# quanpn90/avsr

Measured on AMD Instinct MI355X. Metric: AV-frames/sec/GPU (fwd+bwd) on 15s clips; WER parity on LRS2 test, higher is better.
Workload: dtype bf16

## Files before the change

### avsr_amd/_lib.py

```python
import ctypes
import os

import torch

_HERE = os.path.dirname(os.path.abspath(__file__))
LIB_PATH = os.environ.get("AVSR_LIB_PATH_AB") or os.path.join(_HERE, "libavsr_hip.so")

AVSR_F32, AVSR_BF16 = 0, 1
ACT_NONE, ACT_GELU, ACT_RELU = 0, 1, 2

_c_p = ctypes.c_void_p
_i64 = ctypes.c_int64
_f = ctypes.c_float
_i = ctypes.c_int


class GemmParams(ctypes.Structure):
    _fields_ = [
        ("M", _i), ("N", _i), ("K", _i), ("batch", _i),
        ("dtype", _i), ("a_kmajor", _i), ("b_kmajor", _i), ("c_f32", _i),
        ("A", _c_p), ("lda", _i64), ("strideA", _i64),
        ("B", _c_p), ("ldb", _i64), ("strideB", _i64),
        ("C", _c_p), ("ldc", _i64), ("strideC", _i64),
        ("alpha", _f), ("beta", _f),
# ... 175 lines not shown


class BeamSelectParams(ctypes.Structure):
    _fields_ = [
        ("n", _i), ("V", _i), ("P", _i), ("beam", _i), ("blank", _i), ("eos", _i), ("w_dec", _f), ("w_ctc", _f),
        ("dec", _c_p), ("ld", _i64), ("ids", _c_p), ("psi", _c_p), ("s_prev", _c_p), ("score", _c_p),
        ("out_prev", _c_p), ("out_tok", _c_p), ("out_col", _c_p), ("out_score", _c_p), ("out_dec", _c_p),
        ("out_ctc", _c_p), ("out_s", _c_p), ("nseg", _i), ("seg", _c_p),
    ]


class BeamPostParams(ctypes.Structure):
    _fields_ = [
        ("U", _i), ("beam", _i), ("P", _i), ("R", _i), ("Lmax", _i), ("steps_cap", _i), ("eos", _i),
        ("end_detect", _i), ("d_end", ctypes.c_double), ("pos", _c_p), ("maxlen", _c_p),
        ("sel_prev", _c_p), ("sel_tok", _c_p), ("sel_col", _c_p), ("sel_score", _c_p), ("sel_dec", _c_p),
        ("sel_ctc", _c_p), ("sel_s", _c_p),
        ("tok", _c_p), ("score", _c_p), ("sdec", _c_p), ("sctc", _c_p), ("s_prev", _c_p), ("src", _c_p),
        ("bp_prev", _c_p), ("bp_tok", _c_p), ("end_flag", _c_p), ("end_score", _c_p), ("end_dec", _c_p),
        ("end_ctc", _c_p), ("best_len", _c_p), ("best_end", _c_p), ("done", _c_p),
    ]


class FbankParams(ctypes.Structure):
    _fields_ = [
        ("B", _i), ("T", _i), ("wav", _c_p), ("ldw", _i64), ("n_samples", _c_p),
        ("bins", _i * 28), ("preemph", _f), ("ln_eps", _f), ("out", _c_p),
    ]


class TimeMaskParams(ctypes.Structure):
    _fields_ = [("B", _i), ("L", _i), ("nspan", _i), ("row_bytes", _i64), ("clip_stride_bytes", _i64),
                ("x", _c_p), ("spans", _c_p)]


class AddNoiseParams(ctypes.Structure):
    _fields_ = [("B", _i), ("L", _i), ("x", _c_p), ("ldx", _i64), ("noise", _c_p), ("ldn", _i64),
                ("lengths", _c_p), ("snr_db", _c_p), ("y", _c_p), ("ldy", _i64), ("ws", _c_p)]


class VideoNormParams(ctypes.Structure):
    _fields_ = [
        ("B", _i), ("T", _i), ("H", _i), ("W", _i), ("crop", _i), ("oy", _i), ("ox", _i),
        ("frames", _c_p), ("mean", _f), ("std", _f), ("out", _c_p),
    ]


SYMBOLS = {
    "avsr_version": ([], ctypes.c_char_p),
    "avsr_set_option": ([_i, _i64], _i),
    "avsr_get_option": ([_i], _i64),
    "avsr_gemm": ([ctypes.POINTER(GemmParams), _c_p], _i),
    "avsr_gemm_wgrad_group": ([ctypes.POINTER(GemmParams), _i, _c_p], _i),
    "avsr_gemm_skinny_splits": ([_i, _i, _i], _i),
    "avsr_conv_fwd": ([ctypes.POINTER(ConvParams), _c_p], _i),
    "avsr_conv_bwd_data": ([ctypes.POINTER(ConvParams), _c_p], _i),
    "avsr_conv_bwd_weight": ([ctypes.POINTER(ConvParams), _c_p], _i),
    "avsr_conv_stat_tiles": ([ctypes.POINTER(ConvParams)], _i),
    "avsr_conv_bnr_tiles": ([ctypes.POINTER(ConvParams)], _i),
    "avsr_conv_wgrad_ws": ([ctypes.POINTER(ConvParams)], _i64),
    "avsr_layernorm_fwd": ([ctypes.POINTER(LayerNormParams), _c_p], _i),
    "avsr_layernorm_bwd": ([ctypes.POINTER(LayerNormParams), _c_p], _i),
    "avsr_bn_finalize": ([ctypes.POINTER(BnFinalizeParams), _c_p], _i),
    "avsr_bn_act_fwd": ([ctypes.POINTER(BnActParams), _c_p], _i),
    "avsr_bn_act_bwd_reduce": ([ctypes.POINTER(BnActParams), _c_p], _i),
    "avsr_bn_bwd_apply": ([ctypes.POINTER(BnActParams), _c_p], _i),
    "avsr_stem_pool_fwd": ([ctypes.POINTER(StemPoolParams), _c_p], _i),
    "avsr_stem_pool_bwd_apply": ([ctypes.POINTER(StemPoolParams), _c_p], _i),
    "avsr_bn_bwd_finalize": ([ctypes.POINTER(BnActParams), _i, _c_p], _i),
    "avsr_avgpool_fwd": ([_i, _i, _i, _i, _c_p, _c_p, _c_p], _i),
    "avsr_avgpool_bwd": ([_i, _i, _i, _i, _c_p, _c_p, _c_p], _i),
    "avsr_attn_fwd": ([ctypes.POINTER(AttnParams), _c_p], _i),
    "avsr_debug_attn_stamps": ([_c_p], _i),
    "avsr_attn_bwd_prep": ([ctypes.POINTER(AttnParams), _c_p], _i),
    "avsr_attn_bwd": ([ctypes.POINTER(AttnParams), _c_p], _i),
    "avsr_attn_dropmask": ([ctypes.POINTER(AttnParams), _c_p], _i),
    "avsr_attn_path": ([ctypes.POINTER(AttnParams), _i], _i),
    "avsr_row_lse": ([ctypes.POINTER(XentParams), _c_p], _i),
    "avsr_lsm_fwd": ([ctypes.POINTER(XentParams), _c_p], _i),
    "avsr_lsm_bwd": ([ctypes.POINTER(XentParams), _c_p], _i),
    "avsr_ctc_fwd": ([ctypes.POINTER(CtcParams), _c_p], _i),
    "avsr_ctc_bwd": ([ctypes.POINTER(CtcParams), _c_p], _i),
    "avsr_ctc_align": ([ctypes.POINTER(CtcAlignParams), _c_p], _i),
    "avsr_loss_finalize": ([_i, _c_p, _i, _c_p, _c_p, _f, _i, _c_p, _c_p], _i),
    "avsr_ew_bwd": ([ctypes.POINTER(EwParams), _c_p], _i),
    "avsr_colsum_defer": ([_i], _i),
    "avsr_colsum_flush": ([_c_p], _i),
    "avsr_colsum_inline": ([_i], _i),
    "avsr_dropout_fwd": ([ctypes.POINTER(EwParams), _c_p], _i),
    "avsr_mask_rows": ([_i, _i, _i, _i, _c_p, _i64, _c_p, _c_p], _i),
    "avsr_embed_fwd": ([ctypes.POINTER(EmbedParams), _c_p], _i),
    "avsr_embed_bwd": ([ctypes.POINTER(EmbedParams), _c_p], _i),
    "avsr_cast": ([_i, _i, _i, _i, _c_p, _i64, _c_p, _i64, _f, _f, _c_p], _i),
    "avsr_cast_flat": ([_i, _i, _i64, _c_p, _c_p, _c_p], _i),
    "avsr_stem_pack": ([_i, _i, _i, _c_p, _c_p, _c_p], _i),
    "avsr_stem_wpack": ([_i, _c_p, _c_p, _c_p], _i),
    "avsr_stem_conv_tiles": ([_i, _i], _i),
    "avsr_stem_wpack2": ([_c_p, _c_p, _c_p], _i),
    "avsr_stem_conv_fwd": ([_i, _i, _c_p, _c_p, _c_p, _c_p, _c_p], _i),
    "avsr_stem_wgrad_unpack": ([_c_p, _c_p, _c_p], _i),
    "avsr_audio_pack": ([_i, _i, _i, _i, _c_p, _c_p, _c_p], _i),
    "avsr_weightnorm_fwd": ([_i, _i, _i, _i, _c_p, _c_p, _c_p, _c_p, _c_p], _i),
    "avsr_weightnorm_bwd": ([_i, _i, _i, _c_p, _c_p, _c_p, _c_p, _c_p, _c_p, _c_p, _c_p], _i),
    "avsr_sumsq": ([_c_p, _i64, _c_p, _c_p, _c_p], _i),
    "avsr_adamw": ([ctypes.POINTER(AdamWParams), _c_p], _i),
    "avsr_log_softmax_rows": ([_i, _i, _i, _c_p, _i64, _c_p, _i64, _c_p], _i),
    "avsr_dec_attn": ([ctypes.POINTER(DecAttnParams), _c_p], _i),
    "avsr_row_topk": ([ctypes.POINTER(TopkParams), _c_p], _i),
    "avsr_log_softmax_topk": ([_i, _i, _i, _c_p, _i64, _c_p, _i64, _i, _c_p, _c_p], _i),
    "avsr_ctc_prefix": ([ctypes.POINTER(CtcPrefixParams), _c_p], _i),
    "avsr_beam_select": ([ctypes.POINTER(BeamSelectParams), _c_p], _i),
    "avsr_beam_step_prep": ([_i, _i, _c_p, _c_p, _c_p, _c_p], _i),
    "avsr_beam_kv_put": ([_i, _i, _i, _c_p, _i64, _c_p, _c_p, _c_p, _c_p], _i),
    "avsr_beam_post": ([ctypes.POINTER(BeamPostParams), _c_p], _i),
    "avsr_gather_rows": ([_i, _i, _i64, _c_p, _i64, _i64, _c_p, _i64, _i64, _c_p, _c_p], _i),
    "avsr_fbank_stack": ([ctypes.POINTER(FbankParams), _c_p], _i),
    "avsr_video_normalize": ([ctypes.POINTER(VideoNormParams), _c_p], _i),
    "avsr_time_mask": ([ctypes.POINTER(TimeMaskParams), _c_p], _i),
    "avsr_add_noise": ([ctypes.POINTER(AddNoiseParams), _c_p], _i),
    "avsr_rgb_to_gray": ([_c_p, _c_p, _i64, _c_p], _i),
}

_lib = None


class AvsrLibError(RuntimeError):
    pass


def load():
    global _lib
    if _lib is not None:
        return _lib
    if not os.path.exists(LIB_PATH):
        raise AvsrLibError(f"{LIB_PATH} not built: run `python -c 'import __graft_entry__ as g; g.build()'`")
    lib = ctypes.CDLL(LIB_PATH, mode=ctypes.RTLD_GLOBAL)
    for name, (argtypes, restype) in SYMBOLS.items():
        if os.environ.get("AVSR_LIB_PATH_AB") and not hasattr(lib, name):
            continue
        fn = getattr(lib, name)
        fn.argtypes = argtypes
        fn.restype = restype
    _lib = lib
    return lib


def check(rc, op):
    if rc != 0:
        raise AvsrLibError(f"{op} failed with code {rc}")


OPTIONS = {"gemm_tile": 0, "attn_sq_fwd": 1, "attn_sq_bwd": 2, "wgrad_dual": 3, "conv_192": 4, "conv_s2phase": 5,
           "conv_patch": 6, "conv_wpatch": 7, "stem_pool_2x2": 8,
           "stem_wpatch": 9}
TILES = ["128", "256", "256x128", "128x256", "128s3", "128w8s3", "pp", "192", "192x256", "192w8s3", "64", "64s4"]
ATTN_PATHS = ["f32", "tiled", "resident", "sq", "enc"]


def set_option(name, value):
    if name == "gemm_tile" and not isinstance(value, int):
        value = 0 if value in (None, "auto") else TILES.index(value) + 1
    lib = load()
    prev = get_option(name)
    check(lib.avsr_set_option(OPTIONS[name], int(value)), f"avsr_set_option({name}, {value})")
    return prev


def get_option(name):
    return int(load().avsr_get_option(OPTIONS[name]))


_raw_stream = getattr(torch._C, "_cuda_getCurrentRawStream", None)
_get_device = getattr(torch._C, "_cuda_getDevice", None) or torch.cuda.current_device


def stream_ptr(device=None):
    if _raw_stream is not None:
        idx = _get_device() if device is None else torch.device(device).index
        if idx is None:
            idx = _get_device()
        return ctypes.c_void_p(_raw_stream(idx))
    return ctypes.c_void_p(torch.cuda.current_stream(device).cuda_stream)
```

### avsr_amd/csrc/attention_enc.hip

```cpp
#include "attention.h"

namespace attn {
namespace sq {
constexpr int KT = 64;
constexpr int NS = 3;
constexpr int IMGB = KT * 128;
constexpr int STAGEB = 2 * IMGB;
static_assert(4 * 32 * 65 * 4 <= NS * STAGEB, "store slabs exceed the ring");

typedef __attribute__((address_space(3))) void lds_void_t;

AVSR_DEV int swz(int row) { const int g = (row >> 1) & 7; return g ^ ((g & 1) << 2); }
AVSR_DEV __amdgpu_buffer_rsrc_t rsrc(const void* base, uint32_t bytes) {
  const uint64_t b = (uint64_t)(uintptr_t)base;
  const uint64_t ub = ((uint64_t)(uint32_t)__builtin_amdgcn_readfirstlane((uint32_t)(b >> 32)) << 32) |
                      (uint32_t)__builtin_amdgcn_readfirstlane((uint32_t)b);
  return __builtin_amdgcn_make_buffer_rsrc((void*)(uintptr_t)ub, (short)0, (int)__builtin_amdgcn_readfirstlane(bytes),
                                           0x00020000);
}
AVSR_DEV void dma16(__amdgpu_buffer_rsrc_t r, uint32_t voff, char* lds_wave_base) {
  const uint32_t m = __builtin_amdgcn_readfirstlane((uint32_t)(uintptr_t)(lds_void_t*)lds_wave_base);
  asm volatile("s_mov_b32 m0, %0\n\ts_nop 0\n\tbuffer_load_dwordx4 %1, %2, 0 offen lds" ::"s"(m), "v"(voff), "s"(r)
               : "memory", "m0");
}
// ... 309 lines not shown
  if (g_stamps != nullptr) {
    __syncthreads();
    stamp_part(3, 0);
  }
}

template <int DM>
__global__ __launch_bounds__(NTH) void attn_bwd_dkdv_kernel(AttnArgs a) {
  extern __shared__ __attribute__((aligned(16))) char smem[];
  char* Qs = smem;
  char* dOs = smem + IMG384;
  float* lss = (float*)(smem + 2 * IMG384);
  float* dls = lss + MAXR;
  char* Kw = smem + 2 * IMG384 + 2 * MAXR * 4;
  stamp_part(0, 1);
  const int bh = xcd_id(blockIdx.x, gridDim.x), b = bh / a.H, h = bh % a.H;
  const int tid = threadIdx.x, l = tid & 63, c = l & 31, hh = l >> 5;
  const int w = __builtin_amdgcn_readfirstlane(tid >> 6);
  Kw += w * 4096;
  const int kb0 = w * 32, key = kb0 + c;
  const bf16* Qg = (const bf16*)a.q + (int64_t)b * a.Lq * a.ldq + h * DH;
  const bf16* dOg = (const bf16*)a.dout + (int64_t)b * a.Lq * a.lddo + h * DH;
  const bf16* Kg = (const bf16*)a.k + ((int64_t)b * a.Lk + kb0) * a.ldk + h * DH;
  const bf16* V = (const bf16*)a.v + (int64_t)b * a.Lk * a.ldv + h * DH;
  if (kb0 < a.Lk) {
#pragma unroll
    for (int i = 0; i < 4; ++i) dma_piece(Kg, a.ldk, min(32, a.Lk - kb0), Kw, i, l);
  }
  dma_piece(Qg, a.ldq, a.Lq, Qs, w, l);
  dma_piece(dOg, a.lddo, a.Lq, dOs, w, l);
  {
    const float* f = (w < 6 ? a.lse : a.delta) + (int64_t)bh * a.Lq;
    dma4(rsrc(f, (uint32_t)(a.Lq * 4)), (uint32_t)((64 * (w % 6) + l) * 4), (char*)((w < 6 ? lss : dls) + 64 * (w % 6)));
  }
  bf16x8 vf[4];
#pragma unroll
  for (int s = 0; s < 4; ++s) vf[s] = ldrow_sel(V, a.ldv, key, a.Lk, s * 16 + 8 * hh);
#pragma unroll
  for (int s = 0; s < 4; ++s) asm volatile("" ::"v"(vf[s]));
#pragma unroll
  for (int r = 1; r < 4; ++r) {
    dma_piece(Qg, a.ldq, a.Lq, Qs, 12 * r + w, l);
    dma_piece(dOg, a.lddo, a.Lq, dOs, 12 * r + w, l);
  }
  round_barrier();
  if (tid < MAXR) lss[tid] *= LOG2E;
  const int klen = a.klen ? min(a.klen[b], a.Lk) : a.Lk;
  const bool active = kb0 < klen, kok = key < klen;
  const float sl2 = a.scale * LOG2E;
  const AttnDrop drop(a.drop_p, a.seed, a.B, a.H, a.Lq, a.Lk);
  const float dscale = DM ? drop.scale : 1.f;
  const uint32_t nG = DM == 1 ? drop.npair * GOLD : 0u;
  const uint32_t keyG = DM == 1 ? ((uint32_t)bh * (uint32_t)a.Lq * drop.npair + (uint32_t)(min(key, a.Lk - 1) >> 1)) * GOLD : 0u;
  const bool odd = c & 1;
  const uint64_t* mp = DM == 2 ? a.mq + ((int64_t)bh * a.mnqb * a.mnkb + w) * 16 + ((c & 3) + 4 * (c >> 3)) : nullptr;
  const int mstride = a.mnkb * 16;
  const bool mhi = (c >> 2) & 1;
  const int nt = (a.Lq + 31) >> 5;
  FragOff fo;
  fo.init(l);
  f32x16 dv0, dv1, dk0, dk1;
  zacc(dv0); zacc(dv1); zacc(dk0); zacc(dk1);
#pragma unroll
  for (int r = 0; r < 4; ++r) {
    if (r == 1) vmwait<4>();
    if (r == 2) vmwait<2>();
    if (r == 3) vmwait<0>();
    round_barrier();
    if (r == 0) stamp_part(1, 1);
    if (active) {
#pragma unroll
      for (int u = 0; u < 3; ++u) {
        const int t = 3 * r + u;
        if (t >= nt) break;
        const int qt0 = t * 32;
        uint32_t mbits = 0;
        if (DM == 2) {
          const uint64_t m64 = mp[(int64_t)t * mstride];
          mbits = (mhi ? (uint32_t)(m64 >> 32) : (uint32_t)m64) >> (4 * hh);
        }
        const char* Qt = Qs + t * 4096;
        const char* dOt = dOs + t * 4096;
        f32x16 sc, dp;
        zacc(sc); zacc(dp);
        uint32_t kz = 0;
        asm volatile("" : "+v"(kz));
        const char* Kt = Kw + kz;
#pragma unroll
        for (int s = 0; s < 4; ++s) {
          sc = mfma32(ldA(Qt, fo.row[s]), ldA(Kt, fo.row[s]), sc);
          dp = mfma32(ldA(dOt, fo.row[s]), vf[s], dp);
        }
        if (!(kb0 + 32 <= klen && qt0 + 32 <= a.Lq)) {
#pragma unroll
          for (int e = 0; e < 16; ++e) sc[e] = kok & (qt0 + qrow(e, hh) < a.Lq) ? sc[e] : -INFINITY;
        }
        const uint32_t tG = keyG + (uint32_t)(qt0 + 4 * hh) * nG;
#pragma unroll
        for (int i = 0; i < 4; ++i) {
          const f32x4 ls = *(const f32x4*)&lss[qt0 + 8 * i + 4 * hh];
          const f32x4 ds = *(const f32x4*)&dls[qt0 + 8 * i + 4 * hh];
          bool kb[4] = {true, true, true, true};
          if (DM == 1) {
#pragma unroll
            for (int u = 0; u < 2; ++u) {
              const uint32_t mine = hashG(tG + (uint32_t)(8 * i + (odd ? 2 : 0) + u) * nG, drop.pre);
              const uint32_t other = __shfl_xor(mine, 1, 64);
              const uint32_t h0 = odd ? other : mine, h1 = odd ? mine : other;
              kb[u] = (odd ? (h0 >> 16) : (h0 & 0xFFFFu)) >= drop.thr;
              kb[u + 2] = (odd ? (h1 >> 16) : (h1 & 0xFFFFu)) >= drop.thr;
            }
          }
#pragma unroll
          for (int e = 0; e < 4; ++e) {
            const int r4 = 4 * i + e;
            const float p = fexp2(fmaf(sc[r4], sl2, -ls[e]));
            if (DM == 2) {
              const bool kp = (mbits >> ((r4 & 3) + 8 * (r4 >> 2))) & 1u;
              sc[r4] = kp ? p : 0.f;
              dp[r4] = p * fmaf(kp ? dp[r4] : 0.f, dscale, -ds[e]);
            } else {
              sc[r4] = kb[e] ? p : 0.f;
              dp[r4] = p * fmaf(kb[e] ? dp[r4] : 0.f, dscale, -ds[e]);
            }
          }
        }
        const bf16x8 pa = accb(sc, 0), pb = accb(sc, 1), sa = accb(dp, 0), sb = accb(dp, 1);
        dv0 = mfma32(ldT(dOs, qt0, fo, 0), pa, dv0);
        dv0 = mfma32(ldT(dOs, qt0 + 16, fo, 0), pb, dv0);
        dv1 = mfma32(ldT(dOs, qt0, fo, 1), pa, dv1);
        dv1 = mfma32(ldT(dOs, qt0 + 16, fo, 1), pb, dv1);
        dk0 = mfma32(ldT(Qs, qt0, fo, 0), sa, dk0);
        dk0 = mfma32(ldT(Qs, qt0 + 16, fo, 0), sb, dk0);
        dk1 = mfma32(ldT(Qs, qt0, fo, 1), sa, dk1);
        dk1 = mfma32(ldT(Qs, qt0 + 16, fo, 1), sb, dk1);
      }
    }
  }
  stamp_part(2, 1);
  __syncthreads();
  if (kb0 < a.Lk) {
    float* scr = (float*)smem + w * 32 * 65;
    bf16* DK = (bf16*)a.dk + ((int64_t)b * a.Lk + kb0) * a.lddk + h * DH;
    store_t<bf16>(dk0, dk1, a.scale, scr, DK, a.lddk, a.Lk - kb0);
    bf16* DV = (bf16*)a.dv + ((int64_t)b * a.Lk + kb0) * a.lddv + h * DH;
    store_t<bf16>(dv0, dv1, dscale, scr, DV, a.lddv, a.Lk - kb0);
  }
  if (g_stamps != nullptr) {
    __syncthreads();
    stamp_part(3, 1);
  }
}

constexpr size_t DQ_LDS = 2 * IMG384 > NTH / 64 * 32 * 65 * 4 ? 2 * IMG384 : NTH / 64 * 32 * 65 * 4;
constexpr size_t DKDV_LDS = 3 * IMG384 + 2 * MAXR * 4;
static_assert(DKDV_LDS <= 160 * 1024 && NTH / 64 * 32 * 65 * 4 <= DKDV_LDS, "dK/dV LDS");

template <int DM> void launch(const avsr_attn_params* p, const AttnArgs& a, hipStream_t st) {
  const dim3 g(p->B * p->H);
  if (p->dq_out) {
    allow_lds(attn_bwd_dq_kernel<bf16, DM>);
    hipLaunchKernelGGL((attn_bwd_dq_kernel<bf16, DM>), g, dim3(NTH), DQ_LDS, st, a, (bf16*)p->dq_out, p->lddq_out);
  } else {
    allow_lds(attn_bwd_dq_kernel<float, DM>);
    hipLaunchKernelGGL((attn_bwd_dq_kernel<float, DM>), g, dim3(NTH), DQ_LDS, st, a, p->dq, p->lddq);
  }
  allow_lds(attn_bwd_dkdv_kernel<DM>);
  hipLaunchKernelGGL(attn_bwd_dkdv_kernel<DM>, g, dim3(NTH), DKDV_LDS, st, a);
}
}

int sq_fwd(const avsr_attn_params* p, const AttnArgs& a, hipStream_t st) {
  const int nqb = (p->Lq + 127) / 128;
  const long nwg = (long)p->B * p->H * nqb;
  if (nwg > 0x7fffffffL) return AVSR_E_SHAPE;
  if (a.mq) hipLaunchKernelGGL(sq::attn_fwd_kernel<true>, dim3((unsigned)nwg), dim3(256), sq::NS * sq::STAGEB, st, a, nqb);
  else hipLaunchKernelGGL(sq::attn_fwd_kernel<false>, dim3((unsigned)nwg), dim3(256), sq::NS * sq::STAGEB, st, a, nqb);
  return (int)hipGetLastError();
}

int enc_bwd(const avsr_attn_params* p, const AttnArgs& a, hipStream_t st) {
  if (!(p->drop_p > 0.f)) rb::launch<0>(p, a, st);
  else if (a.mq) rb::launch<2>(p, a, st);
  else rb::launch<1>(p, a, st);
  return (int)hipGetLastError();
}
int enc_stamps(unsigned long long* buf) { return (int)hipMemcpyToSymbol(HIP_SYMBOL(g_stamps), &buf, sizeof(buf)); }
}
```

### avsr_amd/csrc/version.hip

```cpp
#include <atomic>

#include "common.h"

extern "C" const char* avsr_version(void) { return "avsr_hip 0.2.0 gfx950"; }

namespace {
std::atomic<int64_t> g_opt[AVSR_OPT_COUNT] = {{0}, {1}, {0}, {1}, {1}, {1}, {1}, {1}, {1}, {1}};

bool opt_valid(int option, int64_t v) {
  switch (option) {
    case AVSR_OPT_GEMM_TILE: return v >= 0 && v <= AVSR_TILE_COUNT;
    case AVSR_OPT_ATTN_SQ_BWD: return v == 0;
    case AVSR_OPT_ATTN_SQ_FWD:
    case AVSR_OPT_WGRAD_DUAL:
    case AVSR_OPT_CONV_192:
    case AVSR_OPT_CONV_S2PHASE:
    case AVSR_OPT_CONV_PATCH:
    case AVSR_OPT_CONV_WPATCH:
    case AVSR_OPT_STEM_POOL_2X2:
    case AVSR_OPT_STEM_WPATCH: return v == 0 || v == 1;
    default: return false;
  }
}
}

int64_t avsr_opt(int option) { return g_opt[option].load(std::memory_order_relaxed); }

extern "C" int avsr_set_option(int option, int64_t value) {
  if (!opt_valid(option, value)) return AVSR_E_ARG;
  g_opt[option].store(value, std::memory_order_relaxed);
  return 0;
}

extern "C" int64_t avsr_get_option(int option) {
  if (option < 0 || option >= AVSR_OPT_COUNT) return -1;
  return avsr_opt(option);
}
```

### include/avsr_hip.h

```cpp
#ifndef AVSR_HIP_H
#define AVSR_HIP_H

#include <stdint.h>

#ifdef __cplusplus
extern "C" {
#endif

enum { AVSR_F32 = 0, AVSR_BF16 = 1 };
enum { AVSR_ACT_NONE = 0, AVSR_ACT_GELU = 1, AVSR_ACT_RELU = 2 };
enum { AVSR_E_SHAPE = 1001, AVSR_E_ALIGN = 1002, AVSR_E_DTYPE = 1003, AVSR_E_ARG = 1004 };

const char* avsr_version(void);

enum {
  AVSR_OPT_GEMM_TILE = 0,
  AVSR_OPT_ATTN_SQ_FWD = 1,
  AVSR_OPT_ATTN_SQ_BWD = 2,
  AVSR_OPT_WGRAD_DUAL = 3,
  AVSR_OPT_CONV_192 = 4,
  AVSR_OPT_CONV_S2PHASE = 5,
  AVSR_OPT_CONV_PATCH = 6,
  AVSR_OPT_CONV_WPATCH = 7,
  AVSR_OPT_STEM_POOL_2X2 = 8,
  AVSR_OPT_STEM_WPATCH = 9,
  AVSR_OPT_COUNT = 10
};
enum {
  AVSR_TILE_128 = 0, AVSR_TILE_256 = 1, AVSR_TILE_256x128 = 2, AVSR_TILE_128x256 = 3, AVSR_TILE_128s3 = 4,
  AVSR_TILE_128w8s3 = 5, AVSR_TILE_PP = 6, AVSR_TILE_192 = 7, AVSR_TILE_192x256 = 8, AVSR_TILE_192w8s3 = 9,
  AVSR_TILE_64 = 10, AVSR_TILE_64s4 = 11, AVSR_TILE_COUNT = 12
};
int avsr_set_option(int option, int64_t value);
int64_t avsr_get_option(int option);

typedef struct {
  int M, N, K, batch;
  int dtype;
  int a_kmajor, b_kmajor;
  int c_f32;
  const void* A; int64_t lda, strideA;
  const void* B; int64_t ldb, strideB;
  void* C;       int64_t ldc, strideC;
  float alpha, beta;
  const float* bias;
  int act;
  int epi_bwd;
  void* preact;
  const void* res;  int64_t ldr, strideR;
  const void* gate;
  float drop_p;
  uint64_t seed;
  int splitk;
  float* ws;
  float* db;
  float* db_ws;
  unsigned long long* stamp;
  float* skinny_ws;
  const float* ln_c1;
  float ln_eps;
  void* kv_k;
  void* kv_v;
  const int* kv_pos;
  int kv_rows;
  unsigned* slab_cnt;
} avsr_gemm_params;
#define AVSR_GEMM_COLSUM_WS(M, N) ((int64_t)(((M) + 63) / 64) * (N))
#define AVSR_GEMM_SLAB_PAD 1088
#define AVSR_SKINNY_WS (1 << 19)
#define AVSR_SKINNY_CNT 4096
#define AVSR_SLAB_CNT 4096
#define AVSR_SKINNY_WS_BYTES ((int64_t)AVSR_SKINNY_WS * 4 + AVSR_SKINNY_CNT * 4)
#define AVSR_GEMM_SLAB_WS(batch, splitk, M, N) ((int64_t)(batch) * (splitk) * ((int64_t)(M) * (N) + AVSR_GEMM_SLAB_PAD))

int avsr_gemm(const avsr_gemm_params* p, void* stream);
int avsr_gemm_wgrad_group(const avsr_gemm_params* p, int n, void* stream);
int avsr_gemm_skinny_splits(int dtype, int N, int K);

typedef struct {
  int dtype;
  int nimg, hin, win, cin;
  int hout, wout, cout;
  int kh, kw, sh, sw, ph, pw;
  int groups;
  int64_t ldx, ldy;
  const void* x; const void* w; void* y;
  void* dx; const void* dy; float* dw;
  float* stats;
  float alpha, beta;
  int splitk;
  const float* bias; int act; void* preact; const void* res;
  float* ws;
  const void* bnr_h; const void* bnr_res;
  const float* bnr_scale; const float* bnr_shift; const float* bnr_prelu;
  const float* bnr_mean; const float* bnr_invstd;
  const float* bnr_scale2; const float* bnr_shift2; const float* bnr_mean2; const float* bnr_invstd2;
  float* bnr_ws;
} avsr_conv_params;

int avsr_conv_fwd(const avsr_conv_params* p, void* stream);
int avsr_conv_bwd_data(const avsr_conv_params* p, void* stream);
int avsr_conv_bwd_weight(const avsr_conv_params* p, void* stream);
int avsr_conv_stat_tiles(const avsr_conv_params* p);
int avsr_conv_bnr_tiles(const avsr_conv_params* p);
int64_t avsr_conv_wgrad_ws(const avsr_conv_params* p);

typedef struct {
  int dtype, rows, N;
  float eps;
  const void* x; int64_t ldx;
  void* y; int64_t ldy;
  const float* gamma; const float* beta;
  float* mean; float* rstd;
  const void* dy; int64_t lddy;
  void* dx; int64_t lddx;
  const void* dres; int64_t lddres;
  float* dgamma; float* dbeta;
  float* ws;
  void* g; int64_t ldg; float drop_p; uint64_t seed; float* db;
} avsr_layernorm_params;
#define AVSR_LN_BLOCKS 256
#define AVSR_LN_WS(N) (AVSR_LN_BLOCKS * 2 * (N))
#define AVSR_LN_WS3(N) (AVSR_LN_BLOCKS * 3 * (N))
int avsr_layernorm_fwd(const avsr_layernorm_params* p, void* stream);
int avsr_layernorm_bwd(const avsr_layernorm_params* p, void* stream);

typedef struct {
  int tiles, C;
  const float* partials;
  const float* gamma; const float* beta;
  float* running_mean; float* running_var;
  float momentum, eps;
  int training;
  float* mean; float* invstd; float* scale; float* shift;
} avsr_bn_finalize_params;
int avsr_bn_finalize(const avsr_bn_finalize_params* p, void* stream);

typedef struct {
  int dtype, M, C;
  const void* h;
  const float* scale; const float* shift;
  const void* res;
  const float* scale2; const float* shift2;
  const float* prelu;
  void* y;
  const void* dy; void* dz;
  const float* mean; const float* invstd;
  const float* mean2; const float* invstd2;
  float* sums;
  float* dprelu;
  float* dgamma; float* dbeta; float* dgamma2; float* dbeta2;
  void* dh; void* dh2; float beta_acc;
  float* ws;
} avsr_bn_act_params;
#define AVSR_BN_FIN_WS(tiles, C) (((int64_t)(tiles) + ((tiles) > 256 ? ((tiles) + 15) / 16 : 0)) * 4 * (C))
#define AVSR_BN_WS(C) AVSR_BN_FIN_WS(2048, C)
int avsr_bn_act_fwd(const avsr_bn_act_params* p, void* stream);
int avsr_bn_act_bwd_reduce(const avsr_bn_act_params* p, void* stream);
int avsr_bn_bwd_finalize(const avsr_bn_act_params* p, int tiles, void* stream);
int avsr_bn_bwd_apply(const avsr_bn_act_params* p, void* stream);

typedef struct {
  int dtype, nimg, H, W, C, Ho, Wo;
  const void* h; const float* scale; const float* shift; const float* prelu;
  void* y; uint8_t* argmax;
  const void* dy; void* dz;
  const float* mean; const float* invstd;
  float* sums; float* dprelu; float* dgamma; float* dbeta;
  float* ws;
  void* hmax;
  void* dh;
  int64_t m_total;
} avsr_stem_pool_params;
int avsr_stem_pool_fwd(const avsr_stem_pool_params* p, void* stream);
int avsr_stem_pool_bwd_apply(const avsr_stem_pool_params* p, void* stream);

int avsr_avgpool_fwd(int dtype, int nimg, int P, int C, const void* x, void* y, void* stream);
int avsr_avgpool_bwd(int dtype, int nimg, int P, int C, const void* dy, void* dx, void* stream);

// ... 265 lines not shown
```

Measured before the change: 146,900.

## Fuse encoder attention backward dQ and dK/dV into one kernel

Adds a single fused backward kernel for the encoder attention path that computes dK/dV per wave while exchanging dS tiles through LDS so that designated waves compute dQ tiles in the same launch. Q and dO are streamed in double-buffered rounds by DMA, and delta is computed in-kernel. This replaces the separate dQ and dK/dV launches, which each reloaded Q/dO/K and recomputed P. The cost is a more complex schedule with extra LDS and barriers per tile, and dQ work is serialized on two waves per tile. It is enabled by default through a new option.

Result: faster. 148,400, median of 6 (+1.0%).

```diff
diff --git a/avsr_amd/_lib.py b/avsr_amd/_lib.py
--- a/avsr_amd/_lib.py
+++ b/avsr_amd/_lib.py
@@ -351,7 +351,7 @@
 
 OPTIONS = {"gemm_tile": 0, "attn_sq_fwd": 1, "attn_sq_bwd": 2, "wgrad_dual": 3, "conv_192": 4, "conv_s2phase": 5,
            "conv_patch": 6, "conv_wpatch": 7, "stem_pool_2x2": 8,
-           "stem_wpatch": 9}
+           "stem_wpatch": 9, "attn_enc_fused": 10}
 TILES = ["128", "256", "256x128", "128x256", "128s3", "128w8s3", "pp", "192", "192x256", "192w8s3", "64", "64s4"]
 ATTN_PATHS = ["f32", "tiled", "resident", "sq", "enc"]
 
diff --git a/avsr_amd/csrc/attention_enc.hip b/avsr_amd/csrc/attention_enc.hip
--- a/avsr_amd/csrc/attention_enc.hip
+++ b/avsr_amd/csrc/attention_enc.hip
@@ -485,12 +485,268 @@
   }
 }
 
+constexpr int RROWS = NTH / 64 * 8;
+constexpr int RIMG = RROWS * 128;
+constexpr int SLOTB = 2 * RIMG;
+constexpr int XTILE = 32 * 64;
+constexpr int XBUF = NTH / 64 * XTILE;
+constexpr int DQSLAB = 32 * 33 * 4;
+constexpr int F_K = 2 * SLOTB, F_LSE = F_K + IMG384, F_X = F_LSE + 2 * MAXR * 4, F_ST = F_X + 2 * XBUF;
+constexpr size_t FUSED_LDS = F_ST + 2 * DQSLAB;
+static_assert(MAXR == 4 * RROWS && RROWS % 32 == 0 && RROWS % 16 == 0, "four rounds of whole tiles, swizzle period 16");
+static_assert(FUSED_LDS <= 160 * 1024 && NTH / 64 * 32 * 65 * 4 <= FUSED_LDS, "fused backward LDS");
+static_assert(F_X % 16 == 0 && F_ST % 16 == 0, "exchange / slab alignment");
+
+AVSR_DEV uint32_t round_voff(int64_t ld, int w, int l) {
+  const int row = 8 * w + (l >> 3), ch = (l & 7) ^ swz(row);
+  return (uint32_t)((row * ld + ch * 8) * 2);
+}
+AVSR_DEV void dma_round(const bf16* base, int64_t ld, int n, char* img, int r, uint32_t voff, int w) {
+  const int nr = n - RROWS * r;
+  dma16(rsrc(base + (int64_t)RROWS * r * ld, nr > 0 ? (uint32_t)(((nr - 1) * ld + DH) * 2) : 0u), voff, img + w * 1024);
+}
+
+AVSR_DEV uint32_t xoff(int key, int j) { return (uint32_t)(key * 64 + ((j ^ ((key >> 2) & 7)) << 3)); }
+
+template <typename OutT>
+AVSR_DEV void dq_tile(const char* X, const char* Ks, int nkb, int cb, const FragOff& fo, int l, float scale,
+                      float* slab, OutT* out, int64_t ld, int nvalid) {
+  asm volatile("" : "+v"(l));
+  const int c = l & 31, hh = l >> 5, g = (l >> 4) & 1, i = l & 15;
+  const uint32_t kt0 = cb ? fo.tr[1][0] : fo.tr[0][0], kt1 = cb ? fo.tr[1][1] : fo.tr[0][1];
+  uint32_t xo[2][2];
+#pragma unroll
+  for (int S = 0; S < 2; ++S)
+#pragma unroll
+    for (int e = 0; e < 2; ++e) xo[S][e] = xoff(16 * S + 8 * e + 4 * hh + (i >> 2), 4 * g + (i & 3));
+  f32x16 acc;
+  zacc(acc);
+  union Frag { s4v s[2]; bf16x8 x; } ka[2], ds[2];
+  auto read = [&](int kb) {
+    const char* Kb = Ks + kb * 4096;
+    const char* Xb = X + kb * XTILE;
+#pragma unroll
+    for (int S = 0; S < 2; ++S) {
+      ka[S].s[0] = __builtin_amdgcn_ds_read_tr16_b64_v4i16((lds_s4v*)(Kb + S * 2048 + kt0));
+      ka[S].s[1] = __builtin_amdgcn_ds_read_tr16_b64_v4i16((lds_s4v*)(Kb + S * 2048 + kt1));
+      ds[S].s[0] = __builtin_amdgcn_ds_read_tr16_b64_v4i16((lds_s4v*)(Xb + xo[S][0]));
+      ds[S].s[1] = __builtin_amdgcn_ds_read_tr16_b64_v4i16((lds_s4v*)(Xb + xo[S][1]));
+    }
+  };
+  read(0);
+  for (int kb = 0; kb < nkb; ++kb) {
+    const bf16x8 a0 = ka[0].x, b0 = ds[0].x, a1 = ka[1].x, b1 = ds[1].x;
+    read(min(kb + 1, nkb - 1));
+    acc = mfma32(a0, b0, acc);
+    acc = mfma32(a1, b1, acc);
+  }
+#pragma unroll
+  for (int r = 0; r < 16; ++r) slab[c * 33 + qrow(r, hh)] = acc[r] * scale;
+  __builtin_amdgcn_wave_barrier();
+  constexpr int VE = 16 / (int)sizeof(OutT), LPR = 32 / VE, RPI = 64 / LPR;
+  const int rr = l / LPR, ch = (l % LPR) * VE;
+#pragma unroll
+  for (int i0 = 0; i0 < 32; i0 += RPI) {
+    const int q = i0 + rr;
+    if (q < nvalid) {
+      float v[VE];
+#pragma unroll
+      for (int j = 0; j < VE; ++j) v[j] = slab[q * 33 + ch + j];
+      stv(out + (int64_t)q * ld + ch, v);
+    }
+  }
+}
+
+template <typename OutT, int DM>
+__global__ __launch_bounds__(NTH) void attn_bwd_kernel(AttnArgs a, OutT* dq, int64_t lddq) {
+  extern __shared__ __attribute__((aligned(16))) char smem[];
+  char* Ks = smem + F_K;
+  float* lss = (float*)(smem + F_LSE);
+  float* dls = lss + MAXR;
+  stamp_part(0, 0);
+  const int bh = xcd_id(blockIdx.x, gridDim.x), b = bh / a.H, h = bh % a.H;
+  const int tid = threadIdx.x, l = tid & 63, c = l & 31, hh = l >> 5;
+  const int w = __builtin_amdgcn_readfirstlane(tid >> 6);
+  const char* Kw = Ks + w * 4096;
+  const int kb0 = w * 32, key = kb0 + c;
+  const bf16* Qg = (const bf16*)a.q + (int64_t)b * a.Lq * a.ldq + h * DH;
+  const bf16* dOg = (const bf16*)a.dout + (int64_t)b * a.Lq * a.lddo + h * DH;
+  const bf16* Og = (const bf16*)a.o + (int64_t)b * a.Lq * a.ldo + h * DH;
+  const bf16* Kg = (const bf16*)a.k + ((int64_t)b * a.Lk + kb0) * a.ldk + h * DH;
+  const bf16* V = (const bf16*)a.v + (int64_t)b * a.Lk * a.ldv + h * DH;
+  if (kb0 < a.Lk) {
+#pragma unroll
+    for (int i = 0; i < 4; ++i) dma_piece(Kg, a.ldk, min(32, a.Lk - kb0), Ks + w * 4096, i, l);
+  }
+  const uint32_t vq = round_voff(a.ldq, w, l), vdo = round_voff(a.lddo, w, l);
+  dma_round(Qg, a.ldq, a.Lq, smem, 0, vq, w);
+  dma_round(dOg, a.lddo, a.Lq, smem + RIMG, 0, vdo, w);
+  if (w < 6) dma4(rsrc(a.lse + (int64_t)bh * a.Lq, (uint32_t)(a.Lq * 4)), (uint32_t)((64 * w + l) * 4), (char*)(lss + 64 * w));
+  const int qi = kb0 + c;
+  const bool qok = qi < a.Lq;
+  bf16x8 vf[4];
+  float dsum = 0.f;
+  {
+    bf16x8 of[4], ov[4];
+#pragma unroll
+    for (int s = 0; s < 4; ++s) {
+      vf[s] = ldrow_sel(V, a.ldv, key, a.Lk, s * 16 + 8 * hh);
+      of[s] = ldrow_sel(dOg, a.lddo, qi, a.Lq, s * 16 + 8 * hh);
+      ov[s] = ldrow_sel(Og, a.ldo, qi, a.Lq, s * 16 + 8 * hh);
+    }
+#pragma unroll
+    for (int s = 0; s < 4; ++s) asm volatile("" ::"v"(vf[s]), "v"(of[s]), "v"(ov[s]));
+    vmwait<0>();
+#pragma unroll
+    for (int s = 0; s < 4; ++s)
+#pragma unroll
+      for (int j = 0; j < 8; ++j) dsum = fmaf((float)of[s][j], (float)ov[s][j], dsum);
+  }
+  dsum = xor32_sum(dsum);
+  if (hh == 0) {
+    if (qok) a.delta[(int64_t)bh * a.Lq + qi] = dsum;
+    dls[qi] = qok ? dsum : 0.f;
+  }
+  dma_round(Qg, a.ldq, a.Lq, smem + SLOTB, 1, vq, w);
+  dma_round(dOg, a.lddo, a.Lq, smem + SLOTB + RIMG, 1, vdo, w);
+  round_barrier();
+  if (tid < MAXR) lss[tid] *= LOG2E;
+  const int klen = a.klen ? min(a.klen[b], a.Lk) : a.Lk;
+  const bool active = kb0 < klen, kok = key < klen;
+  const int nkb = (klen + 31) >> 5;
+  const float sl2 = a.scale * LOG2E;
+  const AttnDrop drop(a.drop_p, a.seed, a.B, a.H, a.Lq, a.Lk);
+  const float dscale = DM ? drop.scale : 1.f;
+  const uint32_t nG = DM == 1 ? drop.npair * GOLD : 0u;
+  const uint32_t keyG = DM == 1 ? ((uint32_t)bh * (uint32_t)a.Lq * drop.npair + (uint32_t)(min(key, a.Lk - 1) >> 1)) * GOLD : 0u;
+  const bool odd = c & 1;
+  const uint64_t* mp = DM == 2 ? a.mq + ((int64_t)bh * a.mnqb * a.mnkb + w) * 16 + ((c & 3) + 4 * (c >> 3)) : nullptr;
+  const int mstride = a.mnkb * 16;
+  const bool mhi = (c >> 2) & 1;
+  const int nt = (a.Lq + 31) >> 5;
+  FragOff fo;
+  fo.init(l);
+  char* Xw = smem + F_X + w * XTILE;
+  const uint32_t xw = xoff(c, hh);
+  OutT* DQ = dq + (int64_t)b * a.Lq * lddq + h * DH;
+  f32x16 dv0, dv1, dk0, dk1;
+  zacc(dv0); zacc(dv1); zacc(dk0); zacc(dk1);
+  round_barrier();
+  stamp_part(1, 0);
+#pragma unroll
+  for (int t = 0; t < MAXR / 32; ++t) {
+    const int r = t / 3, u = t % 3, qt0 = t * 32;
+    const char* Qs = smem + (r & 1) * SLOTB;
+    const char* dOs = Qs + RIMG;
+    if (active && t < nt) {
+      uint32_t mbits = 0;
+      if (DM == 2) {
+        const uint64_t m64 = mp[(int64_t)t * mstride];
+        mbits = (mhi ? (uint32_t)(m64 >> 32) : (uint32_t)m64) >> (4 * hh);
+      }
+      const char* Qt = Qs + u * 4096;
+      const char* dOt = dOs + u * 4096;
+      f32x16 sc, dp;
+      zacc(sc); zacc(dp);
+      uint32_t kz = 0;
+      asm volatile("" : "+v"(kz));
+      const char* Kt = Kw + kz;
+#pragma unroll
+      for (int s = 0; s < 4; ++s) {
+        sc = mfma32(ldA(Qt, fo.row[s]), ldA(Kt, fo.row[s]), sc);
+        dp = mfma32(ldA(dOt, fo.row[s]), vf[s], dp);
+      }
+      if (!(kb0 + 32 <= klen && qt0 + 32 <= a.Lq)) {
+#pragma unroll
+        for (int e = 0; e < 16; ++e) sc[e] = kok & (qt0 + qrow(e, hh) < a.Lq) ? sc[e] : -INFINITY;
+      }
+      const uint32_t tG = keyG + (uint32_t)(qt0 + 4 * hh) * nG;
+#pragma unroll
+      for (int i = 0; i < 4; ++i) {
+        const f32x4 ls = *(const f32x4*)&lss[qt0 + 8 * i + 4 * hh];
+        const f32x4 ds = *(const f32x4*)&dls[qt0 + 8 * i + 4 * hh];
+        bool kb[4] = {true, true, true, true};
+        if (DM == 1) {
+#pragma unroll
+          for (int u2 = 0; u2 < 2; ++u2) {
+            const uint32_t mine = hashG(tG + (uint32_t)(8 * i + (odd ? 2 : 0) + u2) * nG, drop.pre);
+            const uint32_t other = __shfl_xor(mine, 1, 64);
+            const uint32_t h0 = odd ? other : mine, h1 = odd ? mine : other;
+            kb[u2] = (odd ? (h0 >> 16) : (h0 & 0xFFFFu)) >= drop.thr;
+            kb[u2 + 2] = (odd ? (h1 >> 16) : (h1 & 0xFFFFu)) >= drop.thr;
+          }
+        }
+#pragma unroll
+        for (int e = 0; e < 4; ++e) {
+          const int r4 = 4 * i + e;
+          const float p = fexp2(fmaf(sc[r4], sl2, -ls[e]));
+          if (DM == 2) {
+            const bool kp = (mbits >> ((r4 & 3) + 8 * (r4 >> 2))) & 1u;
+            sc[r4] = kp ? p : 0.f;
+            dp[r4] = p * fmaf(kp ? dp[r4] : 0.f, dscale, -ds[e]);
+          } else {
+            sc[r4] = kb[e] ? p : 0.f;
+            dp[r4] = p * fmaf(kb[e] ? dp[r4] : 0.f, dscale, -ds[e]);
+          }
+        }
+      }
+      const bf16x8 pa = accb(sc, 0), pb = accb(sc, 1), sa = accb(dp, 0), sb = accb(dp, 1);
+      char* Xt = Xw + (t & 1) * XBUF;
+      *(bf16x4*)(Xt + xw) = __builtin_shufflevector(sa, sa, 0, 1, 2, 3);
+      *(bf16x4*)(Xt + (xw ^ 16u)) = __builtin_shufflevector(sa, sa, 4, 5, 6, 7);
+      *(bf16x4*)(Xt + (xw ^ 32u)) = __builtin_shufflevector(sb, sb, 0, 1, 2, 3);
+      *(bf16x4*)(Xt + (xw ^ 48u)) = __builtin_shufflevector(sb, sb, 4, 5, 6, 7);
+      dv0 = mfma32(ldT(dOs, 32 * u, fo, 0), pa, dv0);
+      dv0 = mfma32(ldT(dOs, 32 * u + 16, fo, 0), pb, dv0);
+      dv1 = mfma32(ldT(dOs, 32 * u, fo, 1), pa, dv1);
+      dv1 = mfma32(ldT(dOs, 32 * u + 16, fo, 1), pb, dv1);
+      dk0 = mfma32(ldT(Qs, 32 * u, fo, 0), sa, dk0);
+      dk0 = mfma32(ldT(Qs, 32 * u + 16, fo, 0), sb, dk0);
+      dk1 = mfma32(ldT(Qs, 32 * u, fo, 1), sa, dk1);
+      dk1 = mfma32(ldT(Qs, 32 * u + 16, fo, 1), sb, dk1);
+    }
+    if (u == 2) vmwait<0>();
+    round_barrier();
+    if (u == 2 && r + 2 < 4) {
+      dma_round(Qg, a.ldq, a.Lq, smem + (r & 1) * SLOTB, r + 2, vq, w);
+      dma_round(dOg, a.lddo, a.Lq, smem + (r & 1) * SLOTB + RIMG, r + 2, vdo, w);
+    }
+    const int cb = w - (2 * t) % (NTH / 64);
+    if (t < nt && (cb == 0 || cb == 1))
+      dq_tile<OutT>(smem + F_X + (t & 1) * XBUF, Ks, nkb, cb, fo, l, a.scale, (float*)(smem + F_ST + cb * DQSLAB),
+                    DQ + (int64_t)qt0 * lddq + 32 * cb, lddq, a.Lq - qt0);
+  }
+  stamp_part(2, 0);
+  __syncthreads();
+  {
+    float* scr = (float*)smem + w * 32 * 65;
+    bf16* DK = (bf16*)a.dk + ((int64_t)b * a.Lk + kb0) * a.lddk + h * DH;
+    store_t<bf16>(dk0, dk1, a.scale, scr, DK, a.lddk, a.Lk - kb0);
+    bf16* DV = (bf16*)a.dv + ((int64_t)b * a.Lk + kb0) * a.lddv + h * DH;
+    store_t<bf16>(dv0, dv1, dscale, scr, DV, a.lddv, a.Lk - kb0);
+  }
+  if (g_stamps != nullptr) {
+    __syncthreads();
+    stamp_part(3, 0);
+  }
+}
+
 constexpr size_t DQ_LDS = 2 * IMG384 > NTH / 64 * 32 * 65 * 4 ? 2 * IMG384 : NTH / 64 * 32 * 65 * 4;
 constexpr size_t DKDV_LDS = 3 * IMG384 + 2 * MAXR * 4;
 static_assert(DKDV_LDS <= 160 * 1024 && NTH / 64 * 32 * 65 * 4 <= DKDV_LDS, "dK/dV LDS");
 
 template <int DM> void launch(const avsr_attn_params* p, const AttnArgs& a, hipStream_t st) {
   const dim3 g(p->B * p->H);
+  if (avsr_opt(AVSR_OPT_ATTN_ENC_FUSED) != 0) {
+    if (p->dq_out) {
+      allow_lds(attn_bwd_kernel<bf16, DM>);
+      hipLaunchKernelGGL((attn_bwd_kernel<bf16, DM>), g, dim3(NTH), FUSED_LDS, st, a, (bf16*)p->dq_out, p->lddq_out);
+    } else {
+      allow_lds(attn_bwd_kernel<float, DM>);
+      hipLaunchKernelGGL((attn_bwd_kernel<float, DM>), g, dim3(NTH), FUSED_LDS, st, a, p->dq, p->lddq);
+    }
+    return;
+  }
   if (p->dq_out) {
     allow_lds(attn_bwd_dq_kernel<bf16, DM>);
     hipLaunchKernelGGL((attn_bwd_dq_kernel<bf16, DM>), g, dim3(NTH), DQ_LDS, st, a, (bf16*)p->dq_out, p->lddq_out);
diff --git a/avsr_amd/csrc/version.hip b/avsr_amd/csrc/version.hip
--- a/avsr_amd/csrc/version.hip
+++ b/avsr_amd/csrc/version.hip
@@ -4,8 +4,12 @@
 
 extern "C" const char* avsr_version(void) { return "avsr_hip 0.2.0 gfx950"; }
 
+#ifndef AVSR_AB_ATTN_ENC_FUSED
+#define AVSR_AB_ATTN_ENC_FUSED 1
+#endif
+
 namespace {
-std::atomic<int64_t> g_opt[AVSR_OPT_COUNT] = {{0}, {1}, {0}, {1}, {1}, {1}, {1}, {1}, {1}, {1}};
+std::atomic<int64_t> g_opt[AVSR_OPT_COUNT] = {{0}, {1}, {0}, {1}, {1}, {1}, {1}, {1}, {1}, {1}, {AVSR_AB_ATTN_ENC_FUSED}};
 
 bool opt_valid(int option, int64_t v) {
   switch (option) {
@@ -18,7 +22,8 @@
     case AVSR_OPT_CONV_PATCH:
     case AVSR_OPT_CONV_WPATCH:
     case AVSR_OPT_STEM_POOL_2X2:
-    case AVSR_OPT_STEM_WPATCH: return v == 0 || v == 1;
+    case AVSR_OPT_STEM_WPATCH:
+    case AVSR_OPT_ATTN_ENC_FUSED: return v == 0 || v == 1;
     default: return false;
   }
 }
diff --git a/include/avsr_hip.h b/include/avsr_hip.h
--- a/include/avsr_hip.h
+++ b/include/avsr_hip.h
@@ -24,7 +24,8 @@
   AVSR_OPT_CONV_WPATCH = 7,
   AVSR_OPT_STEM_POOL_2X2 = 8,
   AVSR_OPT_STEM_WPATCH = 9,
-  AVSR_OPT_COUNT = 10
+  AVSR_OPT_ATTN_ENC_FUSED = 10,
+  AVSR_OPT_COUNT = 11
 };
 enum {
   AVSR_TILE_128 = 0, AVSR_TILE_256 = 1, AVSR_TILE_256x128 = 2, AVSR_TILE_128x256 = 3, AVSR_TILE_128s3 = 4,
```
